# kuanyuke/BayHunter

Measured on AMD Instinct MI355X. Metric: forward evals/sec (SWD+RF, 10-layer), higher is better.
Workload: dtype f64; 1 GPU; joint10: rdispph+prf(201 samples, nsamp 512), 10 layers, 21 periods, 524288 models/GPU/step; models_per_gpu=524288, err_models=0, library=bayhunter_amd 0.2 (gfx950) src e081f7e61802b220, overlap=True

## Files before the change

bayhunter_amd/csrc/kernels.hip:

```cpp
#include <hip/hip_runtime.h>
#include <cstdlib>
#include "kernels.h"
#include "rf_core.h"
#include "swd_core.h"
#include "swd_team.h"

namespace bh {

static hipError_t ensure_dyn_lds(const void *func, size_t lds, size_t (&set)[16])
{
    if (lds <= 48 * 1024) return hipSuccess;
    int dev = 0;
    hipError_t e = hipGetDevice(&dev);
    if (e != hipSuccess) return e;
    dev &= 15;
    if (lds > set[dev]) {
        e = hipFuncSetAttribute(func, hipFuncAttributeMaxDynamicSharedMemorySize, (int)lds);
        if (e != hipSuccess) return e;
        set[dev] = lds;
    }
    return hipSuccess;
}

struct LdsLay {
// ... 522 lines not shown
}

struct WideSrc {
    const SwdArgs &A;
    const SwdTargetDev &tg;
    int t, lane, nl, taken;
    long b;
    float *res;
    __device__ __forceinline__ int next(TeamLay &, double *&out, double *&cws, double *&cbws)
    {
        if (taken) return 0;
        taken = 1;
        out = A.out + b * A.out_stride + tg.out_off;
        if (tg.mode > 1) {
            cws = A.ws + ((long)t * 2 * BH_NP) * A.B + b;
            cbws = cws + (long)BH_NP * A.B;
        }
        return nl;
    }
    __device__ __forceinline__ void done(int err)
    {
        if (lane == 0) A.err[b * A.ntargets + t] = err;
        if (lane < tg.nper)
            A.out[b * A.out_stride + tg.out_off + lane] = (double)res[lane];
    }
    __device__ __forceinline__ void put(SwdState &, int k, int, float v) { if (lane == 0) res[k - 1] = v; }
    __device__ __forceinline__ void fill_zero(SwdState &, int k, int kmax)
    {
        if (lane == 0)
            for (int i = k; i <= kmax; i++) res[i - 1] = 0.f;
    }
    __device__ __forceinline__ void sphere(TeamLay &lay, int mmax, int ifunc) { swd_sphere(lay, mmax, ifunc); }
};

template <int W>
__device__ __forceinline__ void swd_teamw_body(const SwdArgs &A)
{
    extern __shared__ double tlds[];
    constexpr int NL = SWD_T * W;
#if defined(BH_TEAM64_LAYERS)
    constexpr bool TPL = false;
#else
    constexpr bool TPL = W == 1;
#endif
    const int lane = threadIdx.x, wl = lane & 63, wave = uni(lane >> 6);
    const bool ctl = W == 1 || wave == 0;
    const int t = blockIdx.y;
    if (!((A.tmask >> t) & 1u)) return;
    const SwdTargetDev tg = A.tg[t];
    const int nm = TPL ? 0 : (A.Lmax > NL ? A.Lmax : NL);
    double *mats = tlds, *dels = mats + swd_mat_off(nm), *perl = dels + SWD_TEAMW_NT, *nevt = perl + BH_NP;
    double *tcl = nevt + 24 * W, *toml = tcl + SWD_TEAMW_NT;
    float *res = (float *)(toml + SWD_TEAMW_NT);
    int *hdr = (int *)(nevt + 24);
    TeamLay lay{res + BH_NP, A.Lmax};
    NevMem nv{nevt, nevt + 12};
    long b = blockIdx.x;
    if (A.order) b = A.order[b];
    const int nl = A.nlay[b];
    if (nl < 1 || nl > A.Lmax) {
        if (lane == 0) swd_bad_depth(A, tg, t, b);
        return;
    }
    {
        const long g = b * A.mstride;
        for (int l = lane; l < nl; l += NL) {
            lay.set_d(l, (float)A.h[g + l]);
            lay.set_a(l, (float)A.vp[g + l]);
            lay.set_b(l, (float)A.vs[g + l]);
            lay.set_rho(l, (float)A.rho[g + l]);
        }
        for (int k = lane; k < tg.nper; k += NL) perl[k] = A.periods[tg.per_off + k];
    }
    __syncthreads();
    WideSrc src{A, tg, t, lane, nl, 0, b, res};
    SwdState S;
    swd_state_init(S);
    TeamwNext nxt{-1, -1, 0.0, 0, 0, 0.0, 0.0, 0.0};
    BH_TP_DECL;
    long rounds = 0;
    bool first = true;
    int cap = 1, ja = 0, ra = 0;
    OneLay mine{0.f, 0.f, 0.f, 0.f}, half{0.f, 0.f, 0.f, 0.f};
    TeamwRound R;
    R.nt = 1; R.nhalf = 0; R.ngrp = 0;
    double mc = 0.0, mom = 0.0;
    for (;;) {
        bool fin = false;
        int nt = 1;
#if defined(BH_TEAMW_USTATE)
        S.c1 = uni(S.c1); S.c2 = uni(S.c2); S.c3 = uni(S.c3); S.del1 = uni(S.del1); S.del2 = uni(S.del2); S.del3 = uni(S.del3);
        S.clow = uni(S.clow); S.del1st = uni(S.del1st); S.ceval = uni(S.ceval); S.omega = uni(S.omega);
        S.cprev = uni(S.cprev); S.ck = uni(S.ck); S.cc = uni(S.cc); S.cfail = uni(S.cfail);
#endif
        if (ctl) {
            if (S.ev != SWD_EV_NONE) swd_driver(S, lay, src, tg, perl, A.B, true);
            fin = S.st == SWD_ST_DONE;
            BH_TP(0);
            if (!fin) {
                if (first) cap = TPL ? (int)SWD_TEAMW_NT : swd_teamw_cap(S.mmax - S.llw, W, tg.iwave);
                R = swd_teamw_round(S, tg, perl, cap, nxt);
                nt = R.nt;
                BH_TP(13);
                swd_teamw_trial(R, S, wl < nt ? wl : 0, &mc, &mom);
                if (lane < nt) { tcl[lane] = mc; toml[lane] = mom; }
            }
            if (W > 1 && lane == 0) { hdr[0] = fin ? 1 : 0; hdr[1] = nt; hdr[2] = S.mmax; hdr[3] = S.llw; }
        }
        __syncthreads();
        if (W > 1 && !ctl) {
            fin = hdr[0] != 0;
            nt = hdr[1];
            S.mmax = hdr[2];
            S.llw = hdr[3];
        }
        if (fin) break;
        BH_TP(1);
        const int nlm = S.mmax - S.llw;
        if (first) {
            first = false;
            cap = TPL ? (int)SWD_TEAMW_NT : swd_teamw_cap(nlm, W, tg.iwave);
            ja = (cap > 1 && nlm > 0) ? lane / nlm : 0;
            ra = lane - ja * nlm;
            const int i0 = S.llw - 1 + (ra < nlm ? ra : 0), ih = S.mmax - 1;
            mine = OneLay{lay.d(i0), lay.a(i0), lay.b(i0), lay.rho(i0)};
            half = OneLay{lay.d(ih), lay.a(ih), lay.b(ih), lay.rho(ih)};
        }
        if (TPL) {
            double dl = 0.0;
            if (wl < nt && mc == mc) {
                const double wvno = mom / mc;
                dl = (tg.iwave == 1) ? swd_dltar1(lay, S.mmax, S.llw, wvno, mom) : swd_dltar4(lay, S.mmax, S.llw, wvno, mom);
            }
            dels[wl] = dl;
            __syncthreads();
            BH_TP(2);
        } else {
            const int jq = 16 * wave + (wl >> 2);
            if (cap > 1) {
                if (ja < nt && nlm > 0) {
                    const double ac = tcl[ja];
                    if (ac == ac)
                        swd_teamw_assemble_one(mine, tg.iwave, S, ra, ac, toml[ja], mats + swd_mat_off(lane));
                }
            } else {
                const double c0 = tcl[0], om0 = toml[0];
                for (int r = lane; r < nlm; r += NL)
                    swd_teamw_assemble_one(lay, tg.iwave, S, r, c0, om0, mats + swd_mat_off(r));
            }
            const bool qvalid = jq < nt;
            const double qc = tcl[qvalid ? jq : 0], qom = toml[qvalid ? jq : 0];
            __syncthreads();
            BH_TP(2);
            if (tg.iwave == 2) {
                if (W == 1 || 16 * wave < nt) {
                    const double del = swd_teamw_chain_quad(lay, half, S, qc, qom, mats, (qvalid ? jq : 0) * nlm);
                    if (qvalid && (wl & 3) == 0) dels[jq] = del;
                }
            } else if (lane < nt) {
                dels[lane] = swd_teamw_chain_one(lay, 1, S, mc, mom, mats, lane * nlm);
            }
            __syncthreads();
        }
        BH_TP(3);
        if (ctl) {
            TeamwNode nd;
            nd.go = SWD_GO_STOP; nd.out = SWD_OUT_CONTROL; nd.c1 = nd.d1 = nd.c2 = nd.d2 = nd.c3n = 0.0;
            unsigned long long goL = 0, goR = 0;
            if (R.nhalf > 0) {
                const bool innode = wl <= R.nhalf;
                nd = swd_teamw_node(S, R, LdsSlots{dels, tcl}, innode ? wl : 0);
                goL = __ballot(innode && nd.go == SWD_GO_LEFT);
                goR = __ballot(innode && nd.go == SWD_GO_RIGHT);
            }
            BH_TP(14);
#if defined(BH_TEAM_PROFILE)
            TeamwVals v{mc, mom, wl < nt ? dels[wl] : 0.0, nt, nd, goL, goR, tp_, &tp_t0_};
#else
            TeamwVals v{mc, mom, wl < nt ? dels[wl] : 0.0, nt, nd, goL, goR};
#endif
            const int used = swd_teamw_consume(S, nv, lay, src, tg, perl, A.B, R, v);
            BH_TP(4);
            BH_TP_COUNT(8, used);
            BH_TP_COUNT(9, nt);
            (void)used;
            rounds++;
        }
    }
    BH_TP_FLUSH(rounds);
    (void)rounds;
}

BH_HD int swd_tpl_team_doubles(int Lmax, int K)
{
    return 7 * K + 24 + (K + 1) / 2 + (4 * Lmax + 1) / 2 + 1;
}

template <int K>
__device__ __forceinline__ void swd_tpl_body(const SwdArgs &A)
{
    extern __shared__ double tlds[];
    static_assert(K == 8 || K == 16 || K == 32, "8, 16 or 32 lanes per search");
    const int sub = threadIdx.x / K, tl = threadIdx.x % K, base = sub * K;
    double *perl = tlds;
    double *mem = tlds + BH_NP + (long)sub * swd_tpl_team_doubles(A.Lmax, K);
    double *tc = mem, *dls = tc + K, *ndc = dls + K, *nevt = ndc + 5 * K;
    int *nout = (int *)(nevt + 24);
    TeamLay lay{(float *)(nevt + 24 + (K + 1) / 2), A.Lmax};
    for (int it = 0; it < A.nsel; it++) {
        const int t = A.tord[it];
        const SwdTargetDev tg = A.tg[t];
        __syncthreads();
        for (int k = threadIdx.x; k < tg.nper; k += SWD_T) perl[k] = A.periods[tg.per_off + k];
        __syncthreads();
        TeamSrc src{A, tg, t, tl, K, 0, (long)blockIdx.x, A.counters + t, nullptr};
        SwdState S;
        swd_state_init(S);
        NevMem nv{nevt, nevt + 12};
        TeamwNext nxt{-1, -1, 0.0, 0, 0, 0.0, 0.0, 0.0};
        TeamwRound R;
        R.nt = 1; R.nhalf = 0; R.ngrp = 0;
        bool live = true;
        for (;;) {
            if (live) {
                if (S.ev != SWD_EV_NONE) swd_driver(S, lay, src, tg, perl, A.B, true);
                live = S.st != SWD_ST_DONE;
            }
            if (!__any(live)) break;
            double mc = __longlong_as_double(0x7ff8000000000000ll), mom = 0.0, dl = 0.0;
            int nt = 0;
            if (live) {
                R = swd_teamw_round(S, tg, perl, K, nxt);
                nt = R.nt;
                if (tl < nt) swd_teamw_trial(R, S, tl, &mc, &mom);
            }
            if (live && tl < nt && mc == mc) {
                const double wvno = mom / mc;
                dl = (tg.iwave == 1) ? swd_dltar1(lay, S.mmax, S.llw, wvno, mom) : swd_dltar4(lay, S.mmax, S.llw, wvno, mom);
            }
            tc[tl] = mc;
            dls[tl] = dl;
            __syncthreads();
            unsigned long long goL = 0, goR = 0;
            {
                const bool innode = live && R.nhalf > 0 && tl <= R.nhalf;
                TeamwNode nd;
                nd.go = SWD_GO_STOP; nd.out = SWD_OUT_CONTROL; nd.c1 = nd.d1 = nd.c2 = nd.d2 = nd.c3n = 0.0;
                if (innode) {
                    nd = swd_teamw_node(S, R, LdsSlots{dls, tc}, tl);
                    nout[tl] = nd.out;
                    ndc[tl] = nd.c1; ndc[K + tl] = nd.d1; ndc[2 * K + tl] = nd.c2; ndc[3 * K + tl] = nd.d2; ndc[4 * K + tl] = nd.c3n;
                }
                goL = (__ballot(innode && nd.go == SWD_GO_LEFT) >> base) & SubVals<K>::MASK;
                goR = (__ballot(innode && nd.go == SWD_GO_RIGHT) >> base) & SubVals<K>::MASK;
            }
            __syncthreads();
            if (live) {
                SubVals<K> v{mc, mom, dl, nt, tl, base, tc, dls, ndc, nout, goL, goR};
                (void)swd_teamw_consume(S, nv, lay, src, tg, perl, A.B, R, v);
            }
            __syncthreads();
        }
    }
}

#define BH_TEAMW_ATTR __attribute__((amdgpu_waves_per_eu(3)))
#if defined(BH_TEAM64_LAYERS)
#define BH_TEAM64_ATTR BH_TEAMW_ATTR
#else
#define BH_TEAM64_ATTR __attribute__((amdgpu_waves_per_eu(3)))
#endif
__global__ __launch_bounds__(SWD_T) BH_TEAM64_ATTR void swd_team_kernel(SwdArgs A) { swd_teamw_body<1>(A); }
__global__ __launch_bounds__(2 * SWD_T) BH_TEAMW_ATTR void swd_team128_kernel(SwdArgs A) { swd_teamw_body<2>(A); }
__global__ __launch_bounds__(4 * SWD_T) BH_TEAMW_ATTR void swd_team256_kernel(SwdArgs A) { swd_teamw_body<4>(A); }
__global__ __launch_bounds__(8 * SWD_T) BH_TEAMW_ATTR void swd_team512_kernel(SwdArgs A) { swd_teamw_body<8>(A); }

#if defined(BH_NARROW_LAYERS)
#define BH_NARROW_BODY swd_team_body
#define BH_NARROW_ATTR __attribute__((amdgpu_waves_per_eu(2, 2)))
#else
#define BH_NARROW_BODY swd_tpl_body
#ifndef BH_NARROW_WAVES
#define BH_NARROW_WAVES 2
#endif
#define BH_NARROW_ATTR __attribute__((amdgpu_waves_per_eu(BH_NARROW_WAVES)))
#endif
__global__ __launch_bounds__(SWD_T) BH_NARROW_ATTR void swd_team32_kernel(SwdArgs A) { BH_NARROW_BODY<32>(A); }
__global__ __launch_bounds__(SWD_T) BH_NARROW_ATTR void swd_team16_kernel(SwdArgs A) { BH_NARROW_BODY<16>(A); }
__global__ __launch_bounds__(SWD_T) BH_NARROW_ATTR void swd_team8_kernel(SwdArgs A) { BH_NARROW_BODY<8>(A); }

__device__ __forceinline__ void rf_block_fft(double *S, int per_model, int Mb, int n, const RfLaunch &P,
                                             const double *tw, int tid)
{
#if !(defined(BH_RF_EXP) && BH_RF_EXP == 1)
    for (int idx = tid; idx < Mb * n; idx += RF_T) {
        int m = idx / n, i = idx - m * n;
        rf_fft_bitrev_scale(S + (long)m * per_model, n, P.log2n, P.sc, i);
    }
    __syncthreads();
#endif
#if defined(BH_RF_EXP) && BH_RF_EXP == 2
    return;
#endif
    for (int l = 1; l < n; l <<= 1) {
        for (int idx = tid; idx < Mb * (n / 2); idx += RF_T) {
            int m = idx / (n / 2), bf = idx - m * (n / 2);
            rf_fft_butterfly(S + (long)m * per_model, tw, l, bf);
        }
        __syncthreads();
    }
}

#ifndef BH_RF_WAVES
#define BH_RF_WAVES 4
#endif
template <bool ZR, bool ROW = false>
__global__ __launch_bounds__(RF_T) __attribute__((amdgpu_waves_per_eu(BH_RF_WAVES, BH_RF_WAVES))) void rf_kernel(RfArgs A)
{
    static_assert(!(ZR && ROW), "the trace form is a single-model call: no per-row slowness");
    extern __shared__ double S[];
    const RfLaunch &P = A.P;
    const int tid = threadIdx.x;
    const int b0 = blockIdx.x * P.M;
    const int Mb = min(P.M, A.B - b0);
    const int L = P.Lmax;
    const RfLayout lo = rf_layout(L, P.nsamp);
    const int n = P.nsamp;
    const int pm = lo.per_model + (ZR ? 4 * P.nfreq : 0);

    for (int idx = tid; idx < Mb * L; idx += RF_T) {
        int m = idx / L, i = idx - m * L;
        long b = b0 + m;
        int nl = A.nlay[b];
        nl = nl < 1 ? 1 : (nl > L ? L : nl);
        if (i < nl)
            rf_phase1_layer(S + (long)m * pm, lo, nl, i, A.h + b * A.mstride,
                            A.vp + b * A.mstride, A.vs + b * A.mstride, A.rho + b * A.mstride,
                            A.qp ? A.qp + b * L : nullptr,
                            A.qs ? A.qs + b * L : nullptr, P.depth_input);
    }
    __syncthreads();
    for (int idx = tid; idx < Mb * L; idx += RF_T) {
        int m = idx / L, i = idx - m * L;
        long b = b0 + m;
        int nl = A.nlay[b];
        nl = nl < 1 ? 1 : (nl > L ? L : nl);
        if (ROW) {
            if (i < nl) {
                bool bad_set;
                const double u = rf_row_slowness(A.set_p, A.set_id, A.nsets, b, &bad_set);
                rf_phase2_interface_at<true>(S + (long)m * pm, lo, P, nl, i, A.vp[b * A.mstride],
                                             A.vs[b * A.mstride], u, u * u);
            }
        } else if (i < nl)
            rf_phase2_interface(S + (long)m * pm, lo, P, nl, i, A.vp[b * A.mstride],
                                A.vs[b * A.mstride]);
    }
    __syncthreads();
#if defined(BH_RF_EXP) && BH_RF_EXP == 3
    const int ntask = 0;
#else
    const int ntask = Mb * P.nact;
#endif
    for (int task = tid; task < ntask; task += RF_T) {
        int m = task / P.nact, j = task - m * P.nact;
        int nl = A.nlay[b0 + m];
        nl = nl < 1 ? 1 : (nl > L ? L : nl);
        double *Sm = S + (long)m * pm;
        const RfFreq F = ROW ? rf_freq_load_lgw(A.ftab, j) : rf_freq_load(A.ftab, j);
        if (ZR) {
            cd zr_r, zr_z;
            cd crf = rf_phase3_task_at<ROW>(Sm, lo, P, nl, j, F, &zr_r, &zr_z);
            rf_xst(Sm, j, crf);
            st_cd(Sm + lo.per_model + 2 * j, zr_r);
            st_cd(Sm + lo.per_model + 2 * P.nfreq + 2 * j, zr_z);
        } else {
            cd crf = rf_phase3_task_at<ROW>(Sm, lo, P, nl, j, F, nullptr, nullptr, A.ftab);
            rf_xst(Sm, j, crf);
        }
    }
    const int nzero = P.nfreq - P.nact;
    for (int idx = tid; idx < Mb * nzero; idx += RF_T) {
        int m = idx / nzero, j = P.nact + (idx - m * nzero);
        double *Sm = S + (long)m * pm;
        rf_xst(Sm, j, mk(0., 0.));
        if (ZR) {
            st_cd(Sm + lo.per_model + 2 * j, mk(0., 0.));
            st_cd(Sm + lo.per_model + 2 * P.nfreq + 2 * j, mk(0., 0.));
        }
    }
    __syncthreads();
    const int nh = n / 2 - 1;
    for (int idx = tid; idx < Mb * nh; idx += RF_T) {
        int m = idx / nh, i = n / 2 + 1 + (idx - m * nh);
        rf_fft_hermitian(S + (long)m * pm, n, i);
    }
    __syncthreads();
    rf_block_fft(S, pm, Mb, n, P, A.tw, tid);
    for (int idx = tid; idx < Mb * P.nout; idx += RF_T) {
        int m = idx / P.nout, i = idx - m * P.nout;
        const int nl = A.nlay[b0 + m];
        const bool bad_depth = nl < 1 || nl > L;
        A.out[(long)(b0 + m) * P.out_stride + P.out_off + i] =
            bad_depth ? __builtin_nan("") : P.qn * S[(long)m * pm + 2 * rf_swz(i)];
    }
    if (ZR) {
        __syncthreads();
        for (int idx = tid; idx < Mb * n; idx += RF_T) {
            int m = idx / n, i = idx - m * n;
            double *Sm = S + (long)m * pm;
            rf_xst(Sm, i, rf_fft_pair_entry(Sm + lo.per_model, Sm + lo.per_model + 2 * P.nfreq, n, i));
        }
        __syncthreads();
        rf_block_fft(S, pm, Mb, n, P, A.tw, tid);
        for (int idx = tid; idx < Mb * n; idx += RF_T) {
            int m = idx / n, i = idx - m * n;
            const double *Sm = S + (long)m * pm;
            const int nl = A.nlay[b0 + m];
            const bool bad_depth = nl < 1 || nl > L;
            A.out_fr[(long)(b0 + m) * n + i] = bad_depth ? __builtin_nan("") : P.qn * Sm[2 * rf_swz(i)];
            A.out_fz[(long)(b0 + m) * n + i] = bad_depth ? __builtin_nan("") : P.qn * Sm[2 * rf_swz(i) + 1];
        }
    }
}

#if defined(BH_TEAM_PROFILE)
extern "C" int bh_debug_team_profile(unsigned long long *out, int reset)
{
    if (out && hipMemcpyFromSymbol(out, HIP_SYMBOL(g_team_prof), sizeof(g_team_prof)) != hipSuccess) return 1;
    if (reset) {
        unsigned long long z[20] = {0};
        if (hipMemcpyToSymbol(HIP_SYMBOL(g_team_prof), z, sizeof(z)) != hipSuccess) return 1;
    }
    return 0;
}
#endif

size_t swd_team_lds_bytes(int Lmax, int team)
{
    if (team >= SWD_T) {
#if defined(BH_TEAM64_LAYERS)
        const int nm = Lmax > team ? Lmax : team;
#else
        const int nm = team == SWD_T ? 0 : (Lmax > team ? Lmax : team);
#endif
        return ((size_t)swd_mat_off(nm) + 3 * SWD_TEAMW_NT + BH_NP + 24 * (team / SWD_T) + BH_NP / 2 + (4 * Lmax + 1) / 2) * sizeof(double);
    }
    const int nsub = SWD_T / team;
#if defined(BH_NARROW_LAYERS)
    const int nm = Lmax > team ? Lmax : team;
    return (size_t)nsub * (nm * SWD_NCA + 2 * SWD_TEAM_NT + (4 * Lmax + 1) / 2) * sizeof(double);
#else
    return ((size_t)BH_NP + (size_t)nsub * swd_tpl_team_doubles(Lmax, team)) * sizeof(double);
#endif
}

static int team_index(int team)
{
    return team == 8 ? 0 : team == 16 ? 1 : team == 32 ? 2 : team == 128 ? 4 : team == 256 ? 5 : team == 512 ? 6 : 3;
}

hipError_t launch_swd_team(const SwdArgs &A, int team, int resident_waves, hipStream_t stream)
{
    if (team != 8 && team != 16 && team != 32 && team != 128 && team != 256 && team != 512) team = 64;
    size_t lds = swd_team_lds_bytes(A.Lmax, team);
    static size_t lds_set[7][16] = {{0}, {0}, {0}, {0}, {0}, {0}, {0}};
    void (*kern)(SwdArgs) = team == 8 ? swd_team8_kernel : team == 16 ? swd_team16_kernel
                          : team == 32 ? swd_team32_kernel : team == 128 ? swd_team128_kernel
                          : team == 256 ? swd_team256_kernel : team == 512 ? swd_team512_kernel : swd_team_kernel;
    hipError_t e = ensure_dyn_lds((const void *)kern, lds, lds_set[team_index(team)]);
    if (e != hipSuccess) return e;
    if (team >= SWD_T) {
        hipLaunchKernelGGL(kern, dim3(A.B, A.ntargets), dim3(team), lds, stream, A);
        return hipGetLastError();
    }
    const int nsub = SWD_T / team;
    int gx = (A.B + nsub - 1) / nsub;
    int per_target = resident_waves / A.nsel;
    if (per_target < 1) per_target = 1;
    if (gx > per_target) gx = per_target;
    hipLaunchKernelGGL(kern, dim3(gx, A.ntargets), dim3(SWD_T), lds, stream, A);
    return hipGetLastError();
}

hipError_t launch_swd(const SwdArgs &A, int resident_waves, hipStream_t stream)
{
    size_t lds = (size_t)4 * A.Lmax * SWD_T * sizeof(float);
    int maxper = 0;
    for (int t = 0; t < A.ntargets; t++)
        if ((A.tmask >> t) & 1u) maxper = A.tg[t].nper > maxper ? A.tg[t].nper : maxper;
    const size_t perbytes = (size_t)BH_NP * sizeof(double);
    const size_t staged = lds + (size_t)maxper * SWD_T * sizeof(float);
    SwdArgs B = A;
    static const bool no_stage = std::getenv("BH_SWD_NO_STAGE") != nullptr;
    B.stage = (!no_stage && maxper > 0 && 8 * (staged + perbytes) <= 160 * 1024) ? maxper : 0;
    if (B.stage) lds = staged;
    lds += perbytes;
    static size_t lds_set[16] = {0};
    hipError_t e0 = ensure_dyn_lds((const void *)swd_kernel, lds, lds_set);
    if (e0 != hipSuccess) return e0;
    int per_target = resident_waves / A.nsel;
    if (per_target < 1) per_target = 1;
    int gx = (A.B + SWD_T - 1) / SWD_T;
    if (gx > 3 * per_target) gx = per_target;
    hipLaunchKernelGGL(swd_kernel, dim3(gx, A.ntargets), dim3(SWD_T), lds, stream, B);
    return hipGetLastError();
}

size_t rf_lds_bytes(int Lmax, int nsamp, int M, bool zr)
{
    RfLayout lo = rf_layout(Lmax, nsamp);
    return (size_t)M * (lo.per_model + (zr ? 4 * (nsamp / 2 + 1) : 0)) * sizeof(double);
}

hipError_t launch_rf(const RfArgs &A, hipStream_t stream)
{
    const bool zr = A.out_fz != nullptr && A.out_fr != nullptr;
    size_t lds = rf_lds_bytes(A.P.Lmax, A.P.nsamp, A.P.M, zr);
    const bool row = A.set_p != nullptr;
    if (row && (zr || A.nsets < 1)) return hipErrorInvalidValue;
    static size_t lds_set[3][16] = {{0}, {0}, {0}};
    void (*kern)(RfArgs) = zr ? rf_kernel<true> : row ? rf_kernel<false, true> : rf_kernel<false>;
    hipError_t e = ensure_dyn_lds((const void *)kern, lds, lds_set[zr ? 1 : row ? 2 : 0]);
    if (e != hipSuccess) return e;
    dim3 grid((A.B + A.P.M - 1) / A.P.M);
    hipLaunchKernelGGL(kern, grid, dim3(RF_T), lds, stream, A);
    return hipGetLastError();
}

}
```

bayhunter_amd/csrc/rf_core.h:

```cpp
#pragma once
#include "bh_common.h"
#include "bh_math.h"

namespace bh {

#ifndef BH_PI
#define BH_PI 3.14159265358979323846
#endif

struct RfLaunch {
    double slowness;
    double p2;
    double gauss;
    double tshift;
    double nsv;
    double sigma;
    double dw;
    double qgauss;
    double sc;
    double qn;
    double wref;
    int nsamp, nfreq, log2n, waveno, nout, out_off, out_stride, Lmax;
    int nact;
    int depth_input;
    int M;
};

enum { RF_REC = 42,
       RF_P_D = 0, RF_P_IVP2 = 1, RF_P_IVS2 = 2,
       RF_P_AP = 3, RF_P_AS = 4,
       RF_P_VP = 5, RF_P_VS = 6, RF_P_RHO = 7,
       RF_P_REAL = 8,
       RF_P_COEF = 9 };
struct RfLayout {
    int L, off_par, off_sc, per_model;
};
BH_HD RfLayout rf_layout(int Lmax, int nsamp)
{
    RfLayout lo;
    int nfreq = nsamp / 2 + 1;
    lo.L = Lmax;
    lo.off_par = 2 * (nfreq + 15);
    lo.off_sc = lo.off_par + RF_REC * Lmax;
    int need = lo.off_sc + 16;
    lo.per_model = need > 2 * nsamp ? need : 2 * nsamp;
#if !defined(BH_RF_NO_PAD)
    lo.per_model += 2;
#endif
    return lo;
}
enum { RF_SC_H2 = 0, RF_SC_T0 = 8, RF_SC_M11 = 9, RF_SC_M12 = 10, RF_SC_M21 = 11, RF_SC_M22 = 12,
       RF_SC_DECOMP = 13, RF_SC_UNIFORM_Q = 14,
       RF_SC_P2 = 15 };

BH_DEV double rf_row_slowness(const double *BH_RESTRICT set_p, const int *BH_RESTRICT set_id, int nsets, long b,
                              bool *bad)
{
    const int s = set_id ? set_id[b] : 0;
    *bad = s < 0 || s >= nsets;
    if (*bad) return __builtin_nan("");
    return set_p[s] * 0.00899;
}

BH_DEV void st_cd(double *p, cd v) { p[0] = v.re; p[1] = v.im; }
BH_DEV cd ld_cd(const double *p) { return mk(p[0], p[1]); }
BH_DEV void st_cm2(double *p, const cm2 &m)
{
    st_cd(p, m.c11); st_cd(p + 2, m.c12); st_cd(p + 4, m.c21); st_cd(p + 6, m.c22);
}
BH_DEV cm2 ld_cm2(const double *p)
{
    cm2 m;
    m.c11 = ld_cd(p); m.c12 = ld_cd(p + 2); m.c21 = ld_cd(p + 4); m.c22 = ld_cd(p + 6);
    return m;
}
BH_DEV cm2 ld_m2(const double *p, const cm2 *) { return ld_cm2(p); }
BH_DEV rm2 ld_m2(const double *p, const rm2 *)
{
    rm2 m;
    m.c11 = p[0]; m.c12 = p[2]; m.c21 = p[4]; m.c22 = p[6];
    return m;
}
BH_DEV cm2 cm2_zero()
{
    cm2 m;
    m.c11 = m.c12 = m.c21 = m.c22 = mk(0.0, 0.0);
    return m;
}

BH_DEV void rf_phase1_layer(double *S, const RfLayout &lo, int nlay, int i, const double *h,
                            const double *vp, const double *vs, const double *rho,
                            const double *qp, const double *qs, int depth_input)
{
    const double R = 6371.0;
    double z, thick;
    if (depth_input) {
        z = h[i];
        thick = (i < nlay - 1) ? h[i + 1] - h[i] : -1.0;
    } else {
        double acc = 0.0;
        for (int k = 0; k < i; k++) acc += h[k];
        z = acc;
        thick = (i < nlay - 1) ? (acc + h[i]) - z : -1.0;
    }
    double lvp = vp[i], lvs = vs[i], lrh = rho[i];
    double zb = z + thick, r = R - z, q = R / r;
    z = R * log(q);
    lvp *= q;
    lvs *= q;
    lrh /= q;
    bool lower_halfspace = !(thick > 0.) && !(lvp < 1. && lrh < 0.1);
    if (!lower_halfspace) {
        r = R - zb;
        q = R / r;
        zb = R * log(q);
        thick = zb - z;
    }
    double *par = S + lo.off_par + RF_REC * i;
    par[RF_P_D] = thick;
    par[RF_P_VP] = lvp;
    par[RF_P_VS] = lvs;
    par[RF_P_RHO] = lrh;
    par[RF_P_AP] = frcp(BH_PI * (qp ? qp[i] : 500.0));
    par[RF_P_AS] = frcp(BH_PI * (qs ? qs[i] : 225.0));
    par[RF_P_IVP2] = frcp(lvp * lvp);
    par[RF_P_IVS2] = frcp(lvs * lvs);
}

BH_DEV void rf_coeffm(double u, double vp1, double vs1, double rho1, double vp2, double vs2,
                      double rho2, cm2 &rd, cm2 &td, cm2 &ru, cm2 &tu)
{
    double mue1 = rho1 * vs1 * vs1, mue2 = rho2 * vs2 * vs2, c = 2. * (mue1 - mue2), u2 = u * u,
           cu2 = c * u2, t1, t2, t3;
    cd rpp, rps, rsp, rss, tpp, tps, tsp, tss, d1, d2, t4, t5, t7;
    cd a1 = conj(csqrt_(mk(1. / (vp1 * vp1) - u2, 0.)));
    cd a2 = conj(csqrt_(mk(1. / (vp2 * vp2) - u2, 0.)));
    cd b1 = conj(csqrt_(mk(1. / (vs1 * vs1) - u2, 0.)));
    cd b2 = conj(csqrt_(mk(1. / (vs2 * vs2) - u2, 0.)));

    t1 = cu2 - rho1 + rho2;
    t2 = cu2 - rho1;
    t3 = cu2 + rho2;
    t4 = a1 * t3 - a2 * t2;

    d1 = (t1 * t1 * u2 + (a2 * (t2 * t2)) * b2) + (a2 * (rho1 * rho2)) * b1;
    d2 = (((a1 * (c * c * u2)) * a2) * b1) * b2 + (a1 * (t3 * t3)) * b1 + (a1 * (rho1 * rho2)) * b2;
    t5 = rdiv(1., d1 + d2);
    t7 = t5 * (2. * rho1);

    rpp = (d2 - d1) * t5;
    rps = ((a1 * (-2. * u)) * t5) * (t1 * t3 + (a2 * (c * t2)) * b2);
    tpp = (a1 * t7) * (b1 * t3 - b2 * t2);
    tps = (((-a1) * t7) * u) * (t1 + (a2 * c) * b1);
    rss = ((d2 - d1) - (a1 * b2 - a2 * b1) * (2. * rho1 * rho2)) * t5;
    rsp = ((b1 * (2. * u)) * t5) * (t1 * t3 + (a2 * (c * t2)) * b2);
    tss = (b1 * t7) * t4;
    tsp = ((b1 * t7) * u) * (t1 + (a1 * c) * b2);
    rd.c11 = rpp; rd.c12 = rsp; rd.c21 = rps; rd.c22 = rss;
    td.c11 = tpp; td.c12 = tsp; td.c21 = tps; td.c22 = tss;

    d1 = (t1 * t1 * u2 + (a1 * (t3 * t3)) * b1) + (a1 * (rho1 * rho2)) * b2;
    d2 = (((a1 * (c * c * u2)) * a2) * b1) * b2 + (a2 * (t2 * t2)) * b2 + (a2 * (rho1 * rho2)) * b1;
    t5 = rdiv(1., d1 + d2);
    t7 = t5 * (2. * rho2);

    rpp = (d2 - d1) * t5;
    rps = ((a2 * (2. * u)) * t5) * (t1 * t2 + (a1 * (c * t3)) * b1);
    tpp = (a2 * t7) * (b1 * t3 - b2 * t2);
    tps = (((-a2) * t7) * u) * (t1 + (a1 * c) * b2);
    rss = ((d2 - d1) - (a2 * b1 - a1 * b2) * (2. * rho1 * rho2)) * t5;
    rsp = ((b2 * (-2. * u)) * t5) * (t1 * t2 + (a1 * (c * t3)) * b1);
    tss = (b2 * t7) * t4;
    tsp = ((b2 * t7) * u) * (t1 + (a2 * c) * b1);
    ru.c11 = rpp; ru.c12 = rsp; ru.c21 = rps; ru.c22 = rss;
    tu.c11 = tpp; tu.c12 = tsp; tu.c21 = tps; tu.c22 = tss;
}

BH_DEV void rf_coeffs(double u, double vp, double vs, cm2 &ru)
{
    double u2 = u * u;
    cd a = csqrt_(mk(1. / (vp * vp) - u2, 0.));
    cd b = csqrt_(mk(1. / (vs * vs) - u2, 0.));
    cd t1 = mk(2. * vs * vs, 0.);
    cd t2 = t1 * u2 - 1.;
    cd d1 = t2 * t2;
    cd d2 = (((t1 * t1) * u2) * a) * b;
    cd d = d1 + d2;
    cd t3 = (((2. * t1) * u) * t2) / d;
    cd rpp = (d2 - d1) / d;
    ru.c11 = rpp; ru.c12 = (-b) * t3; ru.c21 = a * t3; ru.c22 = rpp;
}

BH_DEV cm2 rf_displacement2(double p, double vp, double vs)
{
    double vp2 = vp * vp, vs2 = vs * vs, p2 = p * p, x = 1. - 2. * vs2 * p2;
    cd a1 = conj(csqrt_(mk(1. / vp2 - p2, 0.)));
    cd b1 = conj(csqrt_(mk(1. / vs2 - p2, 0.)));
    cd q = rdiv(1., x * x + (a1 * (4. * vs2 * vs2 * p2)) * b1);
    cm2 m;
    m.c11 = ((((q * a1) * b1) * 2.) * vs2) * p;
    m.c12 = (q * b1) * (1. - 2. * vs2 * p2);
    m.c21 = (q * a1) * (1. - 2. * vs2 * p2);
    m.c22 = (((((-q) * a1) * b1) * 2.) * vs2) * p;
    m.c11 = m.c11 * 2.0; m.c12 = m.c12 * 2.0; m.c21 = m.c21 * 2.0; m.c22 = m.c22 * 2.0;
    return m;
}

template <bool ROW>
BH_DEV void rf_phase2_interface_at(double *S, const RfLayout &lo, const RfLaunch &P, int nlay, int i,
                                   double vp0_in, double vs0_in, const double row_u, const double row_u2)
{
    double *lay = S + lo.off_par;
    double *rec = lay + RF_REC * i, *coef = rec + RF_P_COEF;
    cm2 rd = cm2_zero(), td = cm2_zero(), ru = cm2_zero(), tu = cm2_zero();
    double u = ROW ? row_u : P.slowness;
    if (i == 0) {
        if (ROW) S[lo.off_sc + RF_SC_P2] = row_u2;
        rf_coeffs(u, lay[RF_P_VP], lay[RF_P_VS], ru);
        double *sc = S + lo.off_sc;
        st_cm2(sc + RF_SC_H2, rf_displacement2(u, lay[RF_P_VP], lay[RF_P_VS]));
        double t0 = 0.;
        const double *v = lay + (P.waveno == 0 ? RF_P_VP : RF_P_VS);
        for (int k = 0; k < nlay; k++)
            t0 += lay[RF_REC * k + RF_P_D] * sqrt(1. / (v[RF_REC * k] * v[RF_REC * k]) - (ROW ? row_u2 : P.p2));
        sc[RF_SC_T0] = t0;
        bool uniform = true;
        for (int k = 1; k < nlay - 1; k++)
            uniform = uniform && lay[RF_REC * k + RF_P_AP] == lay[RF_P_AP] && lay[RF_REC * k + RF_P_AS] == lay[RF_P_AS];
        sc[RF_SC_UNIFORM_Q] = uniform ? 1.0 : 0.0;
        double sigma = P.sigma;
        if (!(sigma == sigma)) {
            double vpvs = vp0_in / vs0_in;
            sigma = (2 - vpvs * vpvs) / (2 - 2 * (vpvs * vpvs));
        }
        double nsv = P.nsv > 0 ? P.nsv : vs0_in;
        double vpt = nsv * sqrt((1. - (sigma)) / (.5 - (sigma))), vst = nsv;
        double pp = ROW ? row_u : P.slowness;
        int dec = (vst > 0.01 && fabs(pp) > 0.0001) ? 1 : 0;
        double a = sqrt(1. / (vpt * vpt) - pp * pp), b = sqrt(1. / (vst * vst) - pp * pp);
        sc[RF_SC_M11] = -(2 * vst * vst * pp * pp - 1.) / (vpt * a);
        sc[RF_SC_M12] = 2. * pp * vst * vst / vpt;
        sc[RF_SC_M21] = -2. * pp * vst;
        sc[RF_SC_M22] = (1. - 2. * vst * vst * pp * pp) / (vst * b);
        sc[RF_SC_DECOMP] = (double)dec;
    } else {
        rf_coeffm(u, rec[RF_P_VP - RF_REC], rec[RF_P_VS - RF_REC], rec[RF_P_RHO - RF_REC],
                  rec[RF_P_VP], rec[RF_P_VS], rec[RF_P_RHO], rd, td, ru, tu);
    }
    st_cm2(coef, rd); st_cm2(coef + 8, td); st_cm2(coef + 16, ru); st_cm2(coef + 24, tu);
    const cm2 *four[4] = {&rd, &td, &ru, &tu};
    bool real = true;
    for (int k = 0; k < 4; k++)
        real = real && four[k]->c11.im == 0. && four[k]->c12.im == 0. && four[k]->c21.im == 0. &&
               four[k]->c22.im == 0.;
    rec[RF_P_REAL] = real ? 1.0 : 0.0;
}
BH_DEV void rf_phase2_interface(double *S, const RfLayout &lo, const RfLaunch &P, int nlay, int i,
                                double vp0_in, double vs0_in)
{
    rf_phase2_interface_at<false>(S, lo, P, nlay, i, vp0_in, vs0_in, 0.0, 0.0);
}

struct RfFreq {
    double lgw;
    cd cq;
};
enum { RF_FTAB = 3 };
BH_DEV RfFreq rf_freq_load(const double *BH_RESTRICT ftab, int j)
{
    RfFreq F;
    F.lgw = ftab[RF_FTAB * j];
    F.cq = mk(ftab[RF_FTAB * j + 1], ftab[RF_FTAB * j + 2]);
    return F;
}
BH_DEV RfFreq rf_freq_load_lgw(const double *BH_RESTRICT ftab, int j)
{
    RfFreq F;
    F.lgw = ftab[RF_FTAB * j];
    F.cq = mk(0., 0.);
    return F;
}

#if !defined(BH_HOSTSIM)
#pragma clang fp contract(fast)
#endif
template <class M, bool FIRST>
BH_DEV void rf_layer_step(const double *ci, const double *cn, cd e11, cd e22, cm2 &m, cm2 &t, cm2 &g)
{
    const M ru = ld_m2(ci + 16, (const M *)nullptr);
    if (FIRST) {
        m.c11 = cmul(ru.c11, e11); m.c12 = cmul(ru.c12, e11);
        m.c21 = cmul(ru.c21, e22); m.c22 = cmul(ru.c22, e22);
    } else {
        const M td = ld_m2(ci + 8, (const M *)nullptr);
        cm2 w;
        w.c11 = cmadd(cmul(m.c11, t.c11), m.c12, t.c21); w.c12 = cmadd(cmul(m.c11, t.c12), m.c12, t.c22);
        w.c21 = cmadd(cmul(m.c21, t.c11), m.c22, t.c21); w.c22 = cmadd(cmul(m.c21, t.c12), m.c22, t.c22);
        cm2 nt;
        nt.c11 = cmadd(cmadd(ru.c11, td.c11, w.c11), td.c12, w.c21);
        nt.c12 = cmadd(cmadd(ru.c12, td.c11, w.c12), td.c12, w.c22);
        nt.c21 = cmadd(cmadd(ru.c21, td.c21, w.c11), td.c22, w.c21);
        nt.c22 = cmadd(cmadd(ru.c22, td.c21, w.c12), td.c22, w.c22);
        m.c11 = cmul(e11, nt.c11); m.c12 = cmul(e11, nt.c12);
        m.c21 = cmul(e22, nt.c21); m.c22 = cmul(e22, nt.c22);
    }
    cm2 nb;
    nb.c11 = cmul(m.c11, e11); nb.c12 = cmul(m.c12, e22); nb.c21 = cmul(m.c21, e11); nb.c22 = cmul(m.c22, e22);
    const M rd = ld_m2(cn, (const M *)nullptr), tu = ld_m2(cn + 24, (const M *)nullptr);
    cm2 x;
    x.c11 = cmsub(cmsub(mk(1., 0.), rd.c11, nb.c11), rd.c12, nb.c21);
    x.c12 = cmsub(cmsub(mk(0., 0.), rd.c11, nb.c12), rd.c12, nb.c22);
    x.c21 = cmsub(cmsub(mk(0., 0.), rd.c21, nb.c11), rd.c22, nb.c21);
    x.c22 = cmsub(cmsub(mk(1., 0.), rd.c21, nb.c12), rd.c22, nb.c22);
    const cd qi = crecip(cmsub(cmul(x.c11, x.c22), x.c12, x.c21));
    const cd p1 = cmul(qi, e11), p2 = cmul(qi, e22);
    cm2 a;
    a.c11 = cmsub(cmul(tu.c11, x.c22), tu.c21, x.c12); a.c12 = cmsub(cmul(tu.c12, x.c22), tu.c22, x.c12);
    a.c21 = cmsub(cmul(tu.c21, x.c11), tu.c11, x.c21); a.c22 = cmsub(cmul(tu.c22, x.c11), tu.c12, x.c21);
    t.c11 = cmul(p1, a.c11); t.c12 = cmul(p1, a.c12); t.c21 = cmul(p2, a.c21); t.c22 = cmul(p2, a.c22);
    if (FIRST) {
        g = t;
    } else {
        cm2 gn;
        gn.c11 = cmadd(cmul(g.c11, t.c11), g.c12, t.c21); gn.c12 = cmadd(cmul(g.c11, t.c12), g.c12, t.c22);
        gn.c21 = cmadd(cmul(g.c21, t.c11), g.c22, t.c21); gn.c22 = cmadd(cmul(g.c21, t.c12), g.c22, t.c22);
        g = gn;
    }
}

template <class M, bool ROW>
BH_DEV cd rf_phase3_body(const double *S, const RfLayout &lo, const RfLaunch &P, int nlay, int j,
                         const RfFreq &F, cd *zr_r, cd *zr_z, const double *BH_RESTRICT ftab)
{
    const double *lay = S + lo.off_par;
    const double *sc = S + lo.off_sc;
    const double row_p2 = ROW ? sc[RF_SC_P2] : 0.0;
    const double w = P.dw * j;
    const double lgw = F.lgw;
    cm2 m = cm2_zero(), tq = cm2_zero(), g = cm2_zero();
    const bool uniform = sc[RF_SC_UNIFORM_Q] != 0.0;
    cd gp, gs;
    {
        const double ap = lay[RF_P_AP], as = lay[RF_P_AS];
        cd fp = mk(1. + lgw * ap, ap * (0.5 * BH_PI)), fs = mk(1. + lgw * as, as * (0.5 * BH_PI));
        gp = crecip(fp * fp);
        gs = crecip(fs * fs);
    }
    for (int i = 0; i < nlay - 1; i++, lay += RF_REC) {
        const double wd = w * lay[RF_P_D];
        if (!uniform && i > 0) {
            const double ap = lay[RF_P_AP], as = lay[RF_P_AS];
            cd fp = mk(1. + lgw * ap, ap * (0.5 * BH_PI)), fs = mk(1. + lgw * as, as * (0.5 * BH_PI));
            gp = crecip(fp * fp);
            gs = crecip(fs * fs);
        }
        cd plc = csqrt_fast(gp * lay[RF_P_IVP2] - (ROW ? row_p2 : P.p2));
        cd slc = csqrt_fast(gs * lay[RF_P_IVS2] - (ROW ? row_p2 : P.p2));
        cd e11 = cexp_bounded(mk(wd * plc.im, -(wd * plc.re))), e22 = cexp_bounded(mk(wd * slc.im, -(wd * slc.re)));
        const double *ci = lay + RF_P_COEF, *cn = ci + RF_REC;
        if (i == 0) rf_layer_step<M, true>(ci, cn, e11, e22, m, tq, g);
        else rf_layer_step<M, false>(ci, cn, e11, e22, m, tq, g);
    }
    cm2 t = ld_cm2(sc + RF_SC_H2) * g;
    cd cr, cz;
    if (P.waveno == 0) { cr = t.c11; cz = t.c21; } else { cr = t.c12; cz = t.c22; }
    if (zr_r) {
        cd qq = cexp_(mk(0., w * sc[RF_SC_T0]));
        cr = cr * qq;
        cz = cz * qq;
    } else {
        const double t0nan = sc[RF_SC_T0] * 0.0;
        cr = cr + mk(t0nan, t0nan);
    }
    if (sc[RF_SC_DECOMP] != 0.0) {
        cd cx = cz * sc[RF_SC_M11] + cr * sc[RF_SC_M12];
        cd cy = cz * sc[RF_SC_M21] + cr * sc[RF_SC_M22];
        cz = cx;
        cr = cy;
    }
    const cd arr_r = cr, arr_z = cz;
    if (P.waveno == 1) { cd tmp = cz; cz = cr; cr = tmp; }
    double denom = cz.re * cz.re + cz.im * cz.im;
    cd crf = (cr * conj(cz)) / denom;
    const cd cq = ROW ? rf_freq_load(ftab, j).cq : F.cq;
    if (zr_r) { *zr_r = arr_r * cq; *zr_z = arr_z * cq; }
#if defined(BH_HOSTSIM)
    return crf * cq;
#else
    return cmul(crf, cq);
#endif
}

template <bool ROW>
BH_DEV cd rf_phase3_task_at(const double *S, const RfLayout &lo, const RfLaunch &P, int nlay, int j,
                            const RfFreq &F, cd *zr_r, cd *zr_z, const double *BH_RESTRICT ftab = nullptr)
{
    const double *flag = S + lo.off_par + RF_P_REAL;
    bool real = true;
    for (int i = 0; i < nlay; i++) real = real && flag[RF_REC * i] != 0.0;
    return real ? rf_phase3_body<rm2, ROW>(S, lo, P, nlay, j, F, zr_r, zr_z, ftab)
                : rf_phase3_body<cm2, ROW>(S, lo, P, nlay, j, F, zr_r, zr_z, ftab);
}
BH_DEV cd rf_phase3_task(const double *S, const RfLayout &lo, const RfLaunch &P, int nlay, int j,
                         const RfFreq &F, cd *zr_r = nullptr, cd *zr_z = nullptr)
{
    return rf_phase3_task_at<false>(S, lo, P, nlay, j, F, zr_r, zr_z);
}

#if !defined(BH_HOSTSIM)
#pragma clang fp contract(off)
#endif

BH_HD int rf_swz(int e) { return e ^ ((e >> 4) & 15); }
BH_DEV cd rf_xld(const double *X, int e) { return ld_cd(X + 2 * rf_swz(e)); }
BH_DEV void rf_xst(double *X, int e, cd v) { st_cd(X + 2 * rf_swz(e), v); }

BH_DEV unsigned rf_bitrev(unsigned i, int log2n)
{
    unsigned r = 0;
    for (int b = 0; b < log2n; b++) { r = (r << 1) | (i & 1u); i >>= 1; }
    return r;
}
BH_DEV void rf_fft_hermitian(double *X, int n, int i)
{
    rf_xst(X, i, conj(rf_xld(X, n - i)));
}
BH_DEV void rf_fft_bitrev_scale(double *X, int n, int log2n, double sc, int i)
{
    int j = (int)rf_bitrev((unsigned)i, log2n);
    if (i > j) return;
    cd xi = rf_xld(X, i), xj = rf_xld(X, j);
    rf_xst(X, j, xi * sc);
    rf_xst(X, i, xj * sc);
    (void)n;
}
BH_DEV cd rf_fft_pair_entry(const double *spec_r, const double *spec_z, int n, int i)
{
    cd c1 = (i <= n / 2) ? ld_cd(spec_r + 2 * i) : conj(ld_cd(spec_r + 2 * (n - i)));
    cd c2 = (i <= n / 2) ? ld_cd(spec_z + 2 * i) : conj(ld_cd(spec_z + 2 * (n - i)));
    return c1 + mk(0., 1.) * c2;
}
BH_DEV void rf_fft_butterfly(double *X, const double *tw, int l, int bf)
{
    int m = bf & (l - 1), i = ((bf - m) << 1) + m;
    cd w = ld_cd(tw + 2 * (l + m));
    cd a = rf_xld(X, i), b = rf_xld(X, i + l);
    cd tmp = w * b;
    rf_xst(X, i + l, a - tmp);
    rf_xst(X, i, a + tmp);
}


}
```

bayhunter_amd/csrc/rf_host.h:

```cpp
#pragma once
#include <cmath>
#include <complex>
#include "rf_core.h"

namespace bh {

constexpr double RF_WEIGHT_CUTOFF = 3.0e-19;

inline void rf_fill_launch(RfLaunch &P, double p, double gauss, int nsamp, double fsamp,
                           double tshift, double nsv, int waveno, int nout)
{
    P.slowness = p * 0.00899;
    P.p2 = P.slowness * P.slowness;
    P.gauss = gauss;
    P.tshift = tshift;
    P.nsv = nsv;
    P.dw = 2.0 * M_PI * fsamp / nsamp;
    P.qgauss = std::sqrt(M_PI) * fsamp / gauss;
    P.sc = std::sqrt(1. / (double)nsamp);
    P.qn = 1. / std::sqrt((double)nsamp);
    P.wref = 2. * M_PI * 1.;
    P.nsamp = nsamp;
    P.nfreq = nsamp / 2 + 1;
    P.log2n = 0;
    while ((1 << P.log2n) < nsamp) P.log2n++;
    P.waveno = waveno;
    P.nout = nout;
    const double wcut = 2.0 * gauss * std::sqrt(std::log(1.0 / RF_WEIGHT_CUTOFF));
    double jcut = std::floor(wcut / P.dw) + 1.0;
    P.nact = (jcut < (double)P.nfreq) ? (int)jcut : P.nfreq;
    if (P.nact < 1) P.nact = 1;
}

inline void rf_fill_freq_table(const RfLaunch &P, double *tab)
{
    for (int j = 0; j < P.nfreq; j++) {
        const double w = P.dw * j;
        tab[RF_FTAB * j] = j ? std::log(w / P.wref) : 0.0;
        double wa = w / P.gauss;
        wa = (wa > 50.0) ? 50.0 : wa;
        const std::complex<double> cq = P.qgauss * std::exp(std::complex<double>(-0.25 * (wa * wa), -w * P.tshift));
        tab[RF_FTAB * j + 1] = cq.real();
        tab[RF_FTAB * j + 2] = cq.imag();
    }
}

inline void rf_fill_twiddles(double *tw, int nsamp)
{
    tw[0] = tw[1] = 0.0;
    for (int l = 1; l < nsamp; l <<= 1)
        for (int m = 0; m < l; m++) {
            std::complex<double> w = std::exp(std::complex<double>(0.0, M_PI * (double)(1 * m) / (double)l));
            tw[2 * (l + m)] = w.real();
            tw[2 * (l + m) + 1] = w.imag();
        }
}

}
```

Before: 9.334 million evals/s.

## Use radix-4 FFT stages and a wave-uniform small-argument exp in RF layer step

Replaces the radix-2 butterfly loop in the block FFT with radix-4 stages, plus a leading radix-2 stage when log2n is odd. This halves the number of LDS passes and __syncthreads barriers. Separately, the per-layer complex exponentials now go through a paired routine that uses a short Taylor polynomial for exp when the whole wavefront has small real arguments, and otherwise falls back to the bounded exp. Also adds host-simulation replay helpers for validation. The polynomial path costs a ballot per call, and its accuracy depends on the threshold.

```diff
diff --git a/bayhunter_amd/csrc/kernels.hip b/bayhunter_amd/csrc/kernels.hip
--- a/bayhunter_amd/csrc/kernels.hip
+++ b/bayhunter_amd/csrc/kernels.hip
@@ -848,10 +848,17 @@
 #if defined(BH_RF_EXP) && BH_RF_EXP == 2
     return;
 #endif
-    for (int l = 1; l < n; l <<= 1) {
+    if (rf_fft_radix2_first(P.log2n)) {
         for (int idx = tid; idx < Mb * (n / 2); idx += RF_T) {
             int m = idx / (n / 2), bf = idx - m * (n / 2);
-            rf_fft_butterfly(S + (long)m * per_model, tw, l, bf);
+            rf_fft_butterfly(S + (long)m * per_model, tw, 1, bf);
+        }
+        __syncthreads();
+    }
+    for (int l = rf_fft_radix4_first(P.log2n); 4 * l <= n; l <<= 2) {
+        for (int idx = tid; idx < Mb * (n / 4); idx += RF_T) {
+            int m = idx / (n / 4), bf = idx - m * (n / 4);
+            rf_fft_butterfly4(S + (long)m * per_model, tw, l, bf);
         }
         __syncthreads();
     }
diff --git a/bayhunter_amd/csrc/rf_core.h b/bayhunter_amd/csrc/rf_core.h
--- a/bayhunter_amd/csrc/rf_core.h
+++ b/bayhunter_amd/csrc/rf_core.h
@@ -281,6 +281,50 @@
     return F;
 }
 
+#define RF_EXP_SMALL 0.34
+#if defined(BH_HOSTSIM) && defined(BH_HOSTSIM_GLIBC_MATH)
+BH_DEV double rf_exp_small(double x) { return std::exp(x); }
+#else
+BH_DEV double rf_exp_small(double x)
+{
+    double p = 1.6059043836821613e-10;
+    p = bh_fma_k(p, x, 2.08767569878681e-09);
+    p = bh_fma_k(p, x, 2.505210838544172e-08);
+    p = bh_fma_k(p, x, 2.755731922398589e-07);
+    p = bh_fma_k(p, x, 2.7557319223985893e-06);
+    p = bh_fma_k(p, x, 2.48015873015873e-05);
+    p = bh_fma_k(p, x, 1.984126984126984e-04);
+    p = bh_fma_k(p, x, 1.3888888888888889e-03);
+    p = bh_fma_k(p, x, 8.333333333333333e-03);
+    p = bh_fma_k(p, x, 4.1666666666666664e-02);
+    p = bh_fma_k(p, x, 1.6666666666666666e-01);
+    p = bh_fma(p, x, 0.5);
+    p = bh_fma(p, x, 1.0);
+    p = bh_fma(p, x, 1.0);
+    return p;
+}
+#endif
+#if defined(BH_HOSTSIM)
+BH_DEV bool rf_wave_all(bool c) { return c; }
+#else
+BH_DEV bool rf_wave_all(bool c) { return __builtin_amdgcn_ballot_w64(!c) == 0ull; }
+#endif
+BH_DEV void rf_cexp_pair(cd za, cd zb, cd *ea, cd *eb)
+{
+    double xa, xb, s, c;
+    if (rf_wave_all(fabs(za.re) <= RF_EXP_SMALL && fabs(zb.re) <= RF_EXP_SMALL)) {
+        xa = rf_exp_small(za.re);
+        xb = rf_exp_small(zb.re);
+    } else {
+        xa = bh_exp_bounded(za.re);
+        xb = bh_exp_bounded(zb.re);
+    }
+    bh_sincos(za.im, &s, &c);
+    *ea = mk(xa * c, xa * s);
+    bh_sincos(zb.im, &s, &c);
+    *eb = mk(xb * c, xb * s);
+}
+
 #if !defined(BH_HOSTSIM)
 #pragma clang fp contract(fast)
 #endif
@@ -356,7 +400,8 @@
         }
         cd plc = csqrt_fast(gp * lay[RF_P_IVP2] - (ROW ? row_p2 : P.p2));
         cd slc = csqrt_fast(gs * lay[RF_P_IVS2] - (ROW ? row_p2 : P.p2));
-        cd e11 = cexp_bounded(mk(wd * plc.im, -(wd * plc.re))), e22 = cexp_bounded(mk(wd * slc.im, -(wd * slc.re)));
+        cd e11, e22;
+        rf_cexp_pair(mk(wd * plc.im, -(wd * plc.re)), mk(wd * slc.im, -(wd * slc.re)), &e11, &e22);
         const double *ci = lay + RF_P_COEF, *cn = ci + RF_REC;
         if (i == 0) rf_layer_step<M, true>(ci, cn, e11, e22, m, tq, g);
         else rf_layer_step<M, false>(ci, cn, e11, e22, m, tq, g);
@@ -449,6 +494,21 @@
     rf_xst(X, i + l, a - tmp);
     rf_xst(X, i, a + tmp);
 }
-
-
-}
+BH_DEV void rf_fft_butterfly4(double *X, const double *tw, int l, int bf)
+{
+    int m = bf & (l - 1), i = ((bf - m) << 2) + m;
+    cd w1 = ld_cd(tw + 2 * (l + m)), w2 = ld_cd(tw + 2 * (2 * l + m)), w3 = ld_cd(tw + 2 * (3 * l + m));
+    cd x0 = rf_xld(X, i), x1 = rf_xld(X, i + l), x2 = rf_xld(X, i + 2 * l), x3 = rf_xld(X, i + 3 * l);
+    cd t1 = w1 * x1, t3 = w1 * x3;
+    cd a0 = x0 + t1, a1 = x0 - t1, a2 = x2 + t3, a3 = x2 - t3;
+    cd u2 = w2 * a2, u3 = w3 * a3;
+    rf_xst(X, i, a0 + u2);
+    rf_xst(X, i + l, a1 + u3);
+    rf_xst(X, i + 2 * l, a0 - u2);
+    rf_xst(X, i + 3 * l, a1 - u3);
+}
+BH_HD bool rf_fft_radix2_first(int log2n) { return (log2n & 1) != 0; }
+BH_HD int rf_fft_radix4_first(int log2n) { return (log2n & 1) ? 2 : 1; }
+
+
+}
diff --git a/bayhunter_amd/csrc/rf_host.h b/bayhunter_amd/csrc/rf_host.h
--- a/bayhunter_amd/csrc/rf_host.h
+++ b/bayhunter_amd/csrc/rf_host.h
@@ -56,4 +56,43 @@
         }
 }
 
+#if defined(BH_HOSTSIM)
+inline void rf_host_fft(double *X, const double *tw, const RfLaunch &P, bool radix4 = true)
+{
+    const int n = P.nsamp;
+    for (int i = 0; i < n; i++) rf_fft_bitrev_scale(X, n, P.log2n, P.sc, i);
+    if (!radix4) {
+        for (int l = 1; l < n; l <<= 1)
+            for (int bf = 0; bf < n / 2; bf++) rf_fft_butterfly(X, tw, l, bf);
+        return;
+    }
+    if (rf_fft_radix2_first(P.log2n))
+        for (int bf = 0; bf < n / 2; bf++) rf_fft_butterfly(X, tw, 1, bf);
+    for (int l = rf_fft_radix4_first(P.log2n); 4 * l <= n; l <<= 2)
+        for (int bf = 0; bf < n / 4; bf++) rf_fft_butterfly4(X, tw, l, bf);
 }
+
+inline void rf_host_replay(int nlay, const double *h, const double *vp, const double *vs, const double *rho,
+                           const double *qp, const double *qs, double p, double gauss, int nsamp, double fsamp,
+                           double tshift, double nsv, int waveno, int nout, double *S, double *tw, double *ftab,
+                           double *rf, bool radix4 = true)
+{
+    RfLaunch P = RfLaunch();
+    rf_fill_launch(P, p, gauss, nsamp, fsamp, tshift, nsv, waveno, nout);
+    P.sigma = std::nan("");
+    P.Lmax = nlay;
+    const RfLayout lo = rf_layout(nlay, nsamp);
+    for (int k = 0; k < lo.per_model; k++) S[k] = 0.0;
+    rf_fill_twiddles(tw, nsamp);
+    rf_fill_freq_table(P, ftab);
+    for (int i = 0; i < nlay; i++) rf_phase1_layer(S, lo, nlay, i, h, vp, vs, rho, qp, qs, 0);
+    for (int i = 0; i < nlay; i++) rf_phase2_interface(S, lo, P, nlay, i, vp[0], vs[0]);
+    for (int j = 0; j < P.nfreq; j++)
+        rf_xst(S, j, j < P.nact ? rf_phase3_task(S, lo, P, nlay, j, rf_freq_load(ftab, j)) : mk(0., 0.));
+    for (int i = nsamp / 2 + 1; i < nsamp; i++) rf_fft_hermitian(S, nsamp, i);
+    rf_host_fft(S, tw, P, radix4);
+    for (int i = 0; i < nout; i++) rf[i] = P.qn * S[2 * rf_swz(i)];
+}
+#endif
+
+}
```

Result: faster. 9.482 million evals/s (median of 6 runs) (+1.6%).
